# o1-labs/proof-systems

Hardware: AMD Instinct MI355X
Metric: MSM Mscalar/s at 2^20 (Vesta) (higher is better)
Workload: dtype u29x9 / u32x8 (255-bit Montgomery integers); 1 GPU; msm_2^20_vesta_srs; points_per_gpu=1048576, points_total=1048576, bases=SRS::<Vesta>::create, scalars=uniform 254-bit, seed 1234+rank, parallelism=point-range x1, world_size_seen=1

## Files before the change

proof_systems_amd/csrc/common.hpp:

```cpp
#pragma once
#include <hip/hip_runtime.h>
#include <stdarg.h>
#include <stdint.h>
#include <stdio.h>
#include <atomic>
#include <chrono>
#include <condition_variable>
#include <initializer_list>
#include <map>
#include <mutex>
#include <set>
#include <string>
#include <thread>
#include <vector>

#include "../../include/kimchi_hip.h"

namespace kh {

void set_error(const char* fmt, ...);

#define KH_HIP(expr)                                                                         \
    do {                                                                                     \
        hipError_t e_ = (expr);                                                              \
// ... 38 lines not shown
    hipEvent_t k0 = nullptr, k1 = nullptr;
    const char* kname = nullptr;
    hipEvent_t ev[MAXP + 1];
    const char* names[MAXP];
    int n = 0;
    bool created = false;
    bool enabled = false;
    int init() {
        if (created) return KH_OK;
        for (int i = 0; i <= MAXP; i++) KH_HIP(hipEventCreate(&ev[i]));
        KH_HIP(hipEventCreate(&k0)); KH_HIP(hipEventCreate(&k1));
        created = true;
        return KH_OK;
    }
    void begin(hipStream_t s) { n = 0; kname = nullptr; if (enabled && created) (void)hipEventRecord(ev[0], s); }
    void mark(const char* name, hipStream_t s) {
        if (!enabled || !created || n >= MAXP) return;
        names[n] = name; n++;
        (void)hipEventRecord(ev[n], s);
    }
};

struct MsmBasis {
    const void* pts = nullptr;
    const uint8_t* inf = nullptr;
    size_t n = 0;
    int precomp_c = 0;
    size_t stride = 0;
    size_t batch_stride = 0;
    const void* wide_pts = nullptr;
    int wide_c = 0;
    bool glv = false;
};

struct MsmJob {
    MsmBasis basis;
    size_t offset = 0;
    const uint64_t* scalars = nullptr;
    size_t n = 0, k = 0;
    int mont = 0, curve = 0;
    int W = 0, c = 0, precomp = 0, planes = 0, plane_shift[2] = {0, 0};
    int wide_lo = 0;
    size_t ngroups = 0;
    bool done_by_flag = false;
    bool fused = false, spread = false;
    bool spread_rerun = false;
};

struct MsmSlot {
    hipStream_t stream = nullptr;
    PhaseTimer timer;
    DevBuf ws_scalars, ws_digits, ws_hist, ws_cnt, ws_off, ws_ntask, ws_toff, ws_entries, ws_partial,
        ws_buckets, ws_seg, ws_out, ws_scan_tmp, ws_biglist, ws_points, ws_order, ws_chunks, ws_handed, ws_sync, ws_mid,
        ws_b29, ws_a1, ws_a2, ws_xlist;
    void* pinned = nullptr; size_t pinned_cap = 0;
    hipEvent_t done = nullptr;
    bool busy = false;
    std::thread::id owner;
    uint64_t ticket = 0;
    MsmJob job;
    volatile uint32_t* host_abort = nullptr;
    volatile uint32_t* spread_abort = nullptr;
    bool flag_unavailable = false;
    bool pinned_coherent = false;
    volatile uint32_t* done_flag = nullptr;
    DevBuf ws_done;
    uint32_t done_expect = 0;
};
static constexpr int MSM_SLOTS = 4;

struct Context {
    std::mutex mu;
    std::condition_variable cv;
    int sync_inflight = 0;
    std::multiset<std::thread::id> blocked_owners;
    int device = -1;
    bool ready = false;
    hipStream_t stream = nullptr;
    bool main_dirty = false;
    hipEvent_t order_ev = nullptr;
    int num_cus = 256;
    size_t lds_per_cu = (size_t)160 << 10, lds_per_block = (size_t)64 << 10;
    bool fused_disabled = false;
    PhaseTimer timer;
    std::vector<std::pair<const char*, float>> last;
    MsmSlot slot[MSM_SLOTS];
    uint64_t next_ticket = 1;
    std::chrono::steady_clock::time_point last_sync_msm_arrival{};
    DevBuf ws_ntt_a, ws_ntt_b;
    void* pinned = nullptr; size_t pinned_cap = 0;
    char* stage = nullptr; size_t stage_cap = 0, stage_cur = 0;
    int stage_upload(void* dst_dev, std::initializer_list<std::pair<const void*, size_t>> parts);
    void mark_async() { if (hipEventRecord(order_ev, stream) == hipSuccess) main_dirty = true; }
    std::mutex scratch_mu;
    std::map<std::string, DevBuf> scratch_bufs;
    std::set<std::string> done_flags;
    DevBuf& scratch(const char* name) { std::lock_guard<std::mutex> lk(scratch_mu); return scratch_bufs[name]; }
    bool once(const char* name) { std::lock_guard<std::mutex> lk(scratch_mu); return done_flags.insert(name).second; }
    void trim_scratch() { std::lock_guard<std::mutex> lk(scratch_mu); for (auto& kv : scratch_bufs) kv.second.release(); }
};
static constexpr int KH_MAX_DEVICES = 16;

Context& ctx();
int ensure_init();
struct DeviceScope {
    int prev;
    explicit DeviceScope(int device);
// ... 11 lines not shown
```

proof_systems_amd/csrc/context.hip:

```cpp
#include <stdlib.h>
#include <algorithm>
#include <atomic>

#include "api_internal.hpp"
#include "env.hpp"

namespace kh {

static thread_local std::string g_err;
void set_error(const char* fmt, ...) {
    char buf[1024];
    va_list ap; va_start(ap, fmt); vsnprintf(buf, sizeof(buf), fmt, ap); va_end(ap);
    g_err = buf;
}

static Context* g_ctx[KH_MAX_DEVICES];
static std::mutex g_ctx_mu;
static int g_default_dev = -1;
static thread_local int tl_dev = -1;
static thread_local int tl_hip_dev = -1;

static thread_local Context* tl_private[KH_MAX_DEVICES];
static std::vector<Context*> g_private_pool[KH_MAX_DEVICES];
static std::atomic<int> g_private_made[KH_MAX_DEVICES];
// ... 174 lines not shown
    return tl.e[d];
}

namespace {
struct DevPool {
    std::mutex mu;
    struct Block { void* p; kh::Context* owner; };
    std::multimap<size_t, Block> free_blocks[KH_MAX_DEVICES];
    std::map<void*, std::pair<int, size_t>> live;
    size_t cached[KH_MAX_DEVICES] = {0};
};
DevPool& dev_pool() { static DevPool p; return p; }
size_t pool_limit() { static const size_t lim = (size_t)env_int("KH_POOL_MAX_MB", 2048) << 20; return lim; }
}
static void dev_pool_trim(int device) {
    DevPool& P = dev_pool();
    std::lock_guard<std::mutex> lk(P.mu);
    const int d = device >= 0 && device < KH_MAX_DEVICES ? device : 0;
    for (auto& kv : P.free_blocks[d]) (void)hipFree(kv.second.p);
    P.free_blocks[d].clear(); P.cached[d] = 0;
}

extern "C" {

int kh_device_count(void) {
    int count = 0;
    if (hipGetDeviceCount(&count) != hipSuccess) return 0;
    return count;
}
int kh_init(int device_id) {
    int rc = do_init(device_id); if (rc) return rc;
    if (device_id >= 0) tl_dev = device_id;
    return KH_OK;
}
int kh_set_device(int device_id) {
    KH_REQUIRE(device_id >= 0, "kh_set_device: negative device id");
    int rc = do_init(device_id); if (rc) return rc;
    tl_dev = device_id;
    return KH_OK;
}
int kh_get_device(void) { return current_device(); }
int kh_trim(void) {
    int rc = ensure_init(); if (rc) return rc;
    Context& C = ctx();
    std::lock_guard<std::mutex> lk(C.mu);
    for (int i = 0; i < MSM_SLOTS; i++) {
        KH_REQUIRE(!C.slot[i].busy, "kh_trim: an MSM is in flight (kh_msm_wait first)");
        KH_HIP(hipStreamSynchronize(C.slot[i].stream));
    }
    for (int i = 0; i < MSM_SLOTS; i++) {
        MsmSlot& S = C.slot[i];
        for (DevBuf* b : {&S.ws_scalars, &S.ws_digits, &S.ws_hist, &S.ws_cnt, &S.ws_off, &S.ws_ntask, &S.ws_toff, &S.ws_entries, &S.ws_partial, &S.ws_buckets,
                          &S.ws_seg, &S.ws_out, &S.ws_scan_tmp, &S.ws_biglist, &S.ws_points, &S.ws_order, &S.ws_chunks, &S.ws_handed, &S.ws_sync, &S.ws_mid,
                          &S.ws_b29, &S.ws_a1, &S.ws_a2, &S.ws_xlist}) b->release();
    }
    C.ws_ntt_a.release(); C.ws_ntt_b.release();
    xfer_trim(C.device);
    dev_pool_trim(C.device);
    C.trim_scratch();
    {
        std::lock_guard<std::mutex> lk2(g_ctx_mu);
        if (g_private_active[C.device >= 0 && C.device < KH_MAX_DEVICES ? C.device : 0] == 0) ntt_trim(C);
    }
    return KH_OK;
}

int kh_private_context_begin(void) {
    int rc = ensure_init(); if (rc) return rc;
    const int dev = current_device();
    KH_REQUIRE(dev >= 0 && dev < KH_MAX_DEVICES, "no current device");
    KH_REQUIRE(!tl_private[dev], "kh_private_context_begin: this thread already has a private context on device %d", dev);
    Context& S = shared_ctx_of(dev);
    Context* c = tl_ctx_cache.c[dev];
    tl_ctx_cache.c[dev] = nullptr;
    if (!c) {
        std::lock_guard<std::mutex> lk(g_ctx_mu);
        if (!g_private_pool[dev].empty()) { c = g_private_pool[dev].back(); g_private_pool[dev].pop_back(); }
    }
    if (!c) {
        c = new (std::nothrow) Context;
        KH_REQUIRE(c, "out of memory");
        g_private_made[dev]++;
    }
    auto give_back = [&](int status) { std::lock_guard<std::mutex> lk(g_ctx_mu); g_private_pool[dev].push_back(c); return status; };
    if ((rc = bind_thread(dev)) || (rc = init_context(*c, dev))) return give_back(rc);
    {
        std::lock_guard<std::mutex> lk(S.mu);
        hipError_t e = hipEventRecord(S.order_ev, S.stream);
        if (e == hipSuccess) e = hipStreamWaitEvent(c->stream, S.order_ev, 0);
        if (e != hipSuccess) { set_error("kh_private_context_begin: ordering behind the shared context failed: %s", hipGetErrorString(e)); return give_back(KH_E_DEVICE); }
    }
    c->mark_async();
    tl_private[dev] = c;
    { std::lock_guard<std::mutex> lk(g_ctx_mu); g_private_active[dev]++; }
    return KH_OK;
}
int kh_set_phase_timers(int on) {
    int rc = ensure_init(); if (rc) return rc;
    Context& C = ctx();
    std::lock_guard<std::mutex> lk(C.mu);
    C.timer.enabled = on != 0; C.timer.n = 0;
    for (int i = 0; i < MSM_SLOTS; i++) { C.slot[i].timer.enabled = on != 0; C.slot[i].timer.n = 0; }
    return KH_OK;
}
int kh_private_context_active(void) {
    const int dev = current_device();
    return dev >= 0 && dev < KH_MAX_DEVICES && tl_private[dev] != nullptr;
// ... 183 lines not shown
```

proof_systems_amd/csrc/msm.hip:

```cpp
#include <hip/hip_ext.h>
#include <math.h>
#include "common.hpp"
#include "env.hpp"
#include "curve.cuh"
#include "coop.cuh"
#include "field29.cuh"
#include "host_ec.hpp"
#include "msm.hpp"
#include <condition_variable>
#include <functional>
#include <memory>
#include <thread>

namespace kh {

#define KH_HIGH_PRIO() __builtin_amdgcn_s_setprio(3)

class HostHelper {
    std::thread th_; std::mutex m_; std::condition_variable cv_, done_cv_;
    std::function<void()> job_; bool has_job_ = false, busy_ = false, stop_ = false;
    void loop() {
        std::unique_lock<std::mutex> lk(m_);
        for (;;) {
            cv_.wait(lk, [&] { return has_job_ || stop_; });
// ... 1257 lines not shown
    }
}
template <class BF>
__global__ void __launch_bounds__(128)
k_marginal_fin_q(const uint8_t* __restrict__ marg, MargGeom g, uint8_t* __restrict__ out, u32* __restrict__ done_ws, u32* __restrict__ done_flag) {
    KH_HIGH_PRIO();
    __shared__ u32 sh[32 * 32];
    const u32 j = blockIdx.x; const size_t q = blockIdx.y;
    const u32 v = threadIdx.x >> 2, role = threadIdx.x & 3u, f = g.wd[j];
    Fe<BF> r = Fe<BF>::zero();
    if (v < (1u << f)) r = quad_load<BF>(marg + ((q * 3 + j) * 32 + v) * 128);
    auto put = [&](const Fe<BF>& x) {
#pragma unroll
        for (int k = 0; k < 8; k++) sh[(v * 4 + role) * 8 + k] = x.v[k];
    };
    auto get = [&](u32 from) {
        Fe<BF> o = Fe<BF>::zero();
        if (from < 32) {
#pragma unroll
            for (int k = 0; k < 8; k++) o.v[k] = sh[(from * 4 + role) * 8 + k];
        }
        return o;
    };
    for (u32 d = 1; d < 32; d <<= 1) {
        put(r); __syncthreads();
        const Fe<BF> o = get(v + d);
        __syncthreads();
        r = quad_add<BF>(r, o);
    }
    if (v == 0 && j != 0) r = Fe<BF>::zero();
    for (u32 d = 16; d >= 1; d >>= 1) {
        put(r); __syncthreads();
        const Fe<BF> o = v < d ? get(v + d) : Fe<BF>::zero();
        __syncthreads();
        r = quad_add<BF>(r, o);
    }
    if (threadIdx.x < 4) quad_store<BF>(out + (q * 3 + j) * 128, r);
    if (done_ws) {
        __threadfence_system();
        __syncthreads();
        if (threadIdx.x == 0) {
            const u32 blocks = gridDim.x * gridDim.y;
            if (__hip_atomic_fetch_add(done_ws, 1u, __ATOMIC_ACQ_REL, __HIP_MEMORY_SCOPE_AGENT) == blocks - 1) {
                __hip_atomic_store(done_ws, 0u, __ATOMIC_RELAXED, __HIP_MEMORY_SCOPE_AGENT);
                const u32 e = done_ws[1] + 1;
                done_ws[1] = e;
                __threadfence_system();
                __hip_atomic_store(done_flag, e, __ATOMIC_RELEASE, __HIP_MEMORY_SCOPE_SYSTEM);
            }
        }
    }
}

struct WideGeom { u32 nb, lo, hi, rlog; };
template <class BF>
__global__ void __launch_bounds__(256)
k_bucket_sum_wide(const u32* __restrict__ toff, const u32* __restrict__ xlist, const u32* __restrict__ slist, const uint8_t* __restrict__ partial,
                  uint8_t* __restrict__ buckets29, u32 low, u32 SMALL_NT, u32* __restrict__ big, u32 cap, uint8_t* __restrict__ chunk_out) {
    KH_HIGH_PRIO();
    __shared__ __attribute__((aligned(16))) uint8_t total[4 * 128];
    const u32 count = xlist[1], nhot = big[0];
    for (u32 it = blockIdx.x * blockDim.x + threadIdx.x; it < count; it += gridDim.x * blockDim.x) {
        const u32 key = slist[it];
        const u32 t0 = toff[key], nt = toff[key + 1] - t0;
        if (nt > SMALL_NT) continue;
        Xyzz<BF> acc = Xyzz<BF>::load(partial + (size_t)t0 * 128);
        for (u32 k = 1; k < nt; k++) acc = add<BF>(acc, Xyzz<BF>::load(partial + (size_t)(t0 + k) * 128));
        uint8_t* const rec = buckets29 + (size_t)wide_true_bucket(key, low) * B29_BYTES;
        if (acc.is_identity()) store_b29_identity<BF>(rec); else store_b29<BF>(rec, xyzz_to29<BF>(acc));
    }
    if (nhot == 0) return;
    const u32 wave = threadIdx.x >> 6, lane = threadIdx.x & 63u, quad = lane >> 2;
    const u32 gw = blockIdx.x * (blockDim.x >> 6) + wave, GW = gridDim.x * (blockDim.x >> 6);
    u32 cbase = 0;
    for (u32 h = 0; h < nhot; h++) {
        const u32 key = big[2 + h];
        const u32 t0 = toff[key], nt = toff[key + 1] - t0, nch = (nt + CHUNK - 1) / CHUNK;
        for (u32 c = (gw + GW - cbase % GW) % GW; c < nch; c += GW) {
            const u32 lo = c * CHUNK, hi = lo + CHUNK < nt ? lo + CHUNK : nt;
            Fe<BF> acc = quad_identity<BF>();
            for (u32 k = lo + quad; k < hi; k += 16) acc = quad_add<BF>(acc, quad_load<BF>(partial + (size_t)(t0 + k) * 128));
            for (int d = 8; d >= 1; d >>= 1) acc = quad_add<BF>(acc, quad_shfl_down<BF>(acc, d));
            if (lane < 4) quad_store<BF>(chunk_out + (size_t)(cbase + c) * 128, acc);
            __threadfence();
            u32 arrived = 0;
            if (lane == 0) arrived = __hip_atomic_fetch_add(&big[2 + cap + h], 1u, __ATOMIC_ACQ_REL, __HIP_MEMORY_SCOPE_AGENT) + 1u;
            arrived = __shfl(arrived, 0, 64);
            if (arrived == nch) {
                __threadfence();
                Fe<BF> o = quad_identity<BF>();
                for (u32 k = quad; k < nch; k += 16) o = quad_add<BF>(o, quad_load<BF>(chunk_out + (size_t)(cbase + k) * 128));
                for (int d = 8; d >= 1; d >>= 1) o = quad_add<BF>(o, quad_shfl_down<BF>(o, d));
                if (lane < 4) quad_store<BF>(total + 128 * wave, o);
                __builtin_amdgcn_wave_barrier();
                if (lane == 0) {
                    const Xyzz<BF> v = Xyzz<BF>::load(total + 128 * wave);
                    uint8_t* const rec = buckets29 + (size_t)wide_true_bucket(key, low) * B29_BYTES;
                    if (v.is_identity()) store_b29_identity<BF>(rec); else store_b29<BF>(rec, xyzz_to29<BF>(v));
                }
                __builtin_amdgcn_wave_barrier();
            }
        }
        cbase += nch;
    }
}
__device__ __forceinline__ void wide_a1_item(const WideGeom& g, u32 out, u32& t0, u32& tstride) {
    const u32 per = g.nb >> g.rlog;
    if (out < per) { t0 = out << g.rlog; tstride = 1u; return; }
    const u32 cpm = (1u << g.hi) >> g.rlog, v = out - per, b = v / cpm, s = v - b * cpm;
    t0 = ((s << g.rlog) << g.lo) + b; tstride = 1u << g.lo;
}
template <class F>
__device__ __forceinline__ bool is_marker29(const Acc29<F>& a) { return a.zz.v[0] == 0xffffffffu; }
template <class BF>
__global__ void __launch_bounds__(256)
k_wide_a1(const uint8_t* __restrict__ buckets29, WideGeom g, u32 ngroups, uint8_t* __restrict__ out29) {
    KH_HIGH_PRIO();
    const u32 per = g.nb >> g.rlog, items = 2u * per;
    const u32 gid = blockIdx.x * blockDim.x + threadIdx.x;
    if (gid >= items * ngroups) return;
    const u32 q = gid / items, u = gid - q * items;
    u32 out = u;
    if (u >= per) { const u32 v = u - per, b = v & ((1u << g.lo) - 1u), sc = v >> g.lo; out = per + b * ((1u << g.hi) >> g.rlog) + sc; }
    u32 t0, ts;
    wide_a1_item(g, out, t0, ts);
    const uint8_t* B = buckets29 + ((size_t)q * g.nb + t0) * B29_BYTES;
    Acc29<BF> acc;
    bool have = false, ok = true;
    const u32 r = 1u << g.rlog;
#pragma unroll 1
    for (u32 i = 0; i < r; i++) {
        const Acc29<BF> b = load_b29<BF>(B + (size_t)i * ts * B29_BYTES);
        if (is_identity29<BF>(b)) continue;
        if (!have) { acc = b; have = true; continue; }
        ok = add29<BF>(acc, b);
        if (!ok) break;
    }
    uint8_t* o = out29 + ((size_t)q * items + out) * B29_BYTES;
    if (!ok) { acc.zz.v[0] = 0xffffffffu; store_b29<BF>(o, acc); return; }
    if (have) store_b29<BF>(o, acc); else store_b29_identity<BF>(o);
}
template <class BF>
__device__ __attribute__((noinline)) Xyzz<BF> wide_chunk_exact(const uint8_t* __restrict__ buckets29g, WideGeom g, u32 out) {
    u32 t0, ts;
    wide_a1_item(g, out, t0, ts);
    Xyzz<BF> acc = Xyzz<BF>::identity();
    const u32 r = 1u << g.rlog;
    for (u32 i = 0; i < r; i++) {
        const Acc29<BF> b = load_b29<BF>(buckets29g + ((size_t)t0 + (size_t)i * ts) * B29_BYTES);
        if (!is_identity29<BF>(b)) acc = add<BF>(acc, xyzz_from29<BF>(b));
    }
    return acc;
}
template <class BF>
__global__ void __launch_bounds__(64)
k_wide_a2(const uint8_t* __restrict__ in29, const uint8_t* __restrict__ buckets29, WideGeom g, uint8_t* __restrict__ outw) {
    KH_HIGH_PRIO();
    __shared__ u32 stage[32][64];
    const u32 slot = blockIdx.x, q = blockIdx.y, plane = slot >> g.lo, sidx = slot & ((1u << g.lo) - 1u);
    const u32 per = g.nb >> g.rlog, items = 2u * per;
    const u32 lane = threadIdx.x, role = lane & 3u, quad = lane >> 2;
    uint8_t* o = outw + (((size_t)q * 2 + plane) * (1u << g.lo) + sidx) * 128;
    u32 cnt, first;
    if (plane == 0) {
        const u32 a = sidx + 1u;
        if (a >= (1u << g.hi)) { if (lane < 4) quad_store<BF>(o, Fe<BF>::zero()); return; }
        cnt = (1u << g.lo) >> g.rlog; first = a * cnt;
    } else { cnt = (1u << g.hi) >> g.rlog; first = per + sidx * cnt; }
    const uint8_t* src = in29 + ((size_t)q * items + first) * B29_BYTES;
    Xyzz<BF> a = Xyzz<BF>::identity();
    for (u32 k = lane; k < cnt; k += 64) {
        const Acc29<BF> b = load_b29<BF>(src + (size_t)k * B29_BYTES);
        if (__builtin_expect(is_marker29<BF>(b), 0)) a = add<BF>(a, wide_chunk_exact<BF>(buckets29 + (size_t)q * g.nb * B29_BYTES, g, first + k));
        else if (!is_identity29<BF>(b)) a = add<BF>(a, xyzz_from29<BF>(b));
    }
#pragma unroll
    for (int k = 0; k < 8; k++) { stage[k][lane] = a.x.v[k]; stage[8 + k][lane] = a.y.v[k]; stage[16 + k][lane] = a.zz.v[k]; stage[24 + k][lane] = a.zzz.v[k]; }
    __syncthreads();
    auto parked = [&](u32 point) {
        Fe<BF> r;
#pragma unroll
        for (int k = 0; k < 8; k++) r.v[k] = stage[role * 8 + k][point];
        return r;
    };
    Fe<BF> acc = parked(quad);
    for (u32 k = 1; k < 4; k++) acc = quad_add<BF>(acc, parked(quad + 16 * k));
    for (int d = 8; d >= 1; d >>= 1) acc = quad_add<BF>(acc, quad_shfl_down<BF>(acc, d));
    if (lane < 4) quad_store<BF>(o, acc);
}

template <class BF>
__global__ void __launch_bounds__(256)
k_precompute(uint8_t* __restrict__ tables, const uint8_t* __restrict__ inf, size_t n, int c, int W, uint8_t* __restrict__ scratch) {
    size_t i = (size_t)blockIdx.x * blockDim.x + threadIdx.x;
    if (i >= n) return;
    if (inf && inf[i]) {
        for (int w = 1; w < W; w++) { Fe<BF> z = Fe<BF>::zero(); z.store(tables + ((size_t)w * n + i) * 64); z.store(tables + ((size_t)w * n + i) * 64 + 32); }
        return;
    }
    Xyzz<BF> P = Xyzz<BF>::from_affine(Aff<BF>::load(tables + i * 64));
    Fe<BF> prod = Fe<BF>::one();
    for (int w = 1; w < W; w++) {
        for (int k = 0; k < c; k++) P = dbl<BF>(P);
        P.store(scratch + ((size_t)(w - 1) * n + i) * 128);
        prod = mul<BF>(prod, P.zzz);
        prod.store(tables + ((size_t)w * n + i) * 64);
    }
    Fe<BF> iv = inv<BF>(prod);
    for (int w = W - 1; w >= 1; w--) {
        Xyzz<BF> Q = Xyzz<BF>::load(scratch + ((size_t)(w - 1) * n + i) * 128);
        Fe<BF> izzz = iv;
        if (w > 1) izzz = mul<BF>(iv, Fe<BF>::load(tables + ((size_t)(w - 1) * n + i) * 64));
        iv = mul<BF>(iv, Q.zzz);
        Fe<BF> izz = sqr<BF>(mul<BF>(izzz, Q.zz));
        Fe<BF> x = mul<BF>(Q.x, izz), y = mul<BF>(Q.y, izzz);
        x.store(tables + ((size_t)w * n + i) * 64);
        y.store(tables + ((size_t)w * n + i) * 64 + 32);
    }
}

struct VestaCfg { typedef FqParams Base; typedef FpParams Scalar; };
struct PallasCfg { typedef FpParams Base; typedef FqParams Scalar; };

static std::atomic<size_t>& wide_min_n_cell() {
    static std::atomic<size_t> v{(size_t)env_int("KH_WIDE_MIN_N", 1 << 19)};
    return v;
}
static std::atomic<u32>& sort_staging_cell(int i) {
    static std::atomic<u32> v[2] = {{(u32)env_int("KH_PART2_STAGE", 28672)}, {(u32)env_int("KH_PART2_MAXPASS", 2)}};
    return v[i];
}
void msm_set_sort_staging(unsigned entries, unsigned max_passes) { sort_staging_cell(0).store(entries); sort_staging_cell(1).store(max_passes); }
size_t msm_wide_min_n() { const size_t v = wide_min_n_cell().load(); return v ? v : ~(size_t)0; }
void msm_set_wide_min_n(size_t n) { wide_min_n_cell().store(n); }
int msm_pick_window(size_t n) {
    int lg = 0; while (((size_t)1 << (lg + 1)) <= n) lg++;
    int c = lg - 3;
    if (c < 4) c = 4;
    if (c > 16) c = 16;
    return c;
}
// ... 26 lines not shown
}

template <class CFG>
static int msm_enqueue_t(Context& Ctx, MsmSlot& C, const MsmBasis& basis, size_t offset, const u64* scalars_dev, size_t n, size_t k,
                         int mont, int curve, int flags) {
    typedef typename CFG::Base BF; typedef typename CFG::Scalar SF;
    hipStream_t s = C.stream;
    const bool wide = basis.wide_pts && basis.wide_c > 16 && basis.wide_c - 9 <= (int)PART2_MAXLOW && n >= msm_wide_min_n() && k <= 4 &&
                      (size_t)windows_of(basis.wide_c) * n <= ((size_t)1 << 26);
    static constexpr u32 SPREAD_MAX_NT = 256;
    const void* const tab_pts = wide ? basis.wide_pts : basis.pts;
    const int c = wide ? basis.wide_c : (basis.precomp_c ? basis.precomp_c : msm_pick_window(n));
    const bool glv = basis.glv && !wide && basis.precomp_c != 0;
    const int W = glv ? 2 * ((128 + c - 1) / c) : windows_of(c);
    const u32 nb = 1u << (c - 1);
    const int precomp = (wide || basis.precomp_c) ? 1 : 0;
    int S = (int)(n / 32768); if (S < 1) S = 1; if (S > 16) S = 16;
    { int want = (int)(512 / ((size_t)W * k)); if (want < 1) want = 1; if (S > want) S = want; }
    const size_t tab_stride = basis.stride ? basis.stride : basis.n;
    SortGeom g{n, nb, S, W, precomp, tab_stride, offset, basis.batch_stride};
    const size_t ngroups = precomp ? k : k * (size_t)W;
    const bool few_groups = ngroups <= 8;
    const bool quad_sum = !wide && precomp && few_groups;
    const bool spread = quad_sum && (flags & MSM_SPREAD_SCALARS) != 0;
    const int Sq = precomp ? W * S : S;
    const size_t nkeys = ngroups * nb;
    const size_t M = n * (size_t)W * k;
    const size_t cap = (size_t)Ctx.num_cus * 256 * 4;
    size_t room_sz = cap / 4;
    if (nkeys < cap / 2) room_sz = cap - cap / 16 - nkeys / 2;
    const u32 room = (u32)room_sz;
    const u32 kmin = 8;
    const KTab ktab = precomp ? task_length_table(nkeys, (u32)Ctx.num_cus) : KTab{};
    const size_t max_tasks = M / 4 + nkeys + 1;
    KH_REQUIRE(M < ((size_t)1 << 31) && (tab_stride * (size_t)(precomp ? W : 1) + basis.batch_stride * k) < ((size_t)1 << 31), "MSM too large for 31-bit entry indices (n=%zu k=%zu)", n, k);

    int rc;
    if ((rc = C.ws_digits.reserve(M * sizeof(int32_t)))) return rc;
    if ((rc = C.ws_hist.reserve(nkeys * Sq * sizeof(u32)))) return rc;
    if ((rc = C.ws_cnt.reserve((nkeys + 2) * sizeof(u32)))) return rc;
    if ((rc = C.ws_off.reserve((nkeys + 2) * sizeof(u32)))) return rc;
    if ((rc = C.ws_ntask.reserve((nkeys + 2) * sizeof(u32)))) return rc;
    if ((rc = C.ws_toff.reserve((nkeys + 2) * sizeof(u32)))) return rc;
    if ((rc = C.ws_entries.reserve((M + 1) * sizeof(u32)))) return rc;
    if ((rc = C.ws_partial.reserve(max_tasks * 128))) return rc;
    if ((rc = C.ws_handed.reserve((max_tasks + 2) * sizeof(u32)))) return rc;
    if ((rc = C.ws_buckets.reserve(nkeys * 128))) return rc;
    const size_t bigcap = nkeys + max_tasks / CHUNK + 2;
    if ((rc = C.ws_biglist.reserve((2 + 4 * bigcap) * sizeof(u32)))) return rc;
    if ((rc = C.ws_chunks.reserve(bigcap * 128))) return rc;
    if ((rc = C.ws_order.reserve((2 * (MAX_K + 1) + 3 * (nkeys + 2)) * sizeof(u32)))) return rc;
    WideGeom wg{};
    static constexpr u32 wide_og = 16, wide_acc_blocks = 3, wide_rlog = 4;
    static_assert((wide_og & (wide_og - 1)) == 0 && wide_og <= (1u << (17 - 9)) && wide_rlog >= 1 && wide_rlog <= 17 / 2, "wide-path constants");
    size_t wide_acc_lds = (Ctx.lds_per_cu / (wide_acc_blocks + 1) + 1024) & ~(size_t)1023;
    if (wide_acc_lds > Ctx.lds_per_block) wide_acc_lds = Ctx.lds_per_block & ~(size_t)1023;
    if (wide) {
        if ((rc = C.ws_xlist.reserve((3 * max_tasks + 8) * sizeof(u32)))) return rc;
        if ((rc = C.ws_handed.reserve((2 * max_tasks + 4) * sizeof(u32)))) return rc;
        wg.nb = nb; wg.lo = (u32)c / 2; wg.hi = (u32)(c - 1) - wg.lo; wg.rlog = wide_rlog;
        if ((rc = C.ws_b29.reserve(nkeys * B29_BYTES))) return rc;
        if ((rc = C.ws_a1.reserve(ngroups * 2 * (size_t)(nb >> wg.rlog) * B29_BYTES))) return rc;
        if ((rc = C.ws_a2.reserve(ngroups * 2 * ((size_t)1 << wg.lo) * 128))) return rc;
    }
    u32 m = 1;
    while (m < 16 && (ngroups * (size_t)nb) / m > 65536) m <<= 1;
    if (!precomp && m < 4) m = 4;
    if (nb < m) m = nb;
    const u32 nseg = nb / m;
    const u32 nblk1 = (nseg + SUM_BLK - 1) / SUM_BLK;
    const u32 planes = wide ? 3u : ((precomp && ngroups <= 4096 && c >= 7 && c <= 16) ? 3u : 0u);
    MargGeom mg{};
    if (planes) {
        const u32 bits = wide ? wg.lo : (u32)c - 1, f0 = (bits + 2) / 3, f1 = (bits - f0 + 1) / 2, f2 = bits - f0 - f1;
        mg.nb = wide ? 1u << wg.lo : nb; mg.sh[0] = 0; mg.wd[0] = f0; mg.sh[1] = f0; mg.wd[1] = f1; mg.sh[2] = f0 + f1; mg.wd[2] = f2;
    }
    const size_t tail_groups = wide ? 2 * ngroups : ngroups;
    const size_t nout = planes ? tail_groups * planes : ngroups;
    if ((rc = C.ws_seg.reserve(std::max(ngroups * (size_t)(nseg + nblk1), nout * (size_t)32) * 128))) return rc;
    if ((rc = C.ws_out.reserve(nout * 128))) return rc;
    if (C.pinned_cap < nout * 128) {
        if (C.pinned) (void)hipHostFree(C.pinned);
        C.pinned = nullptr; C.pinned_cap = 0;
        C.pinned_coherent = hipHostMalloc(&C.pinned, nout * 128 + 4096, hipHostMallocCoherent | hipHostMallocMapped) == hipSuccess;
        if (!C.pinned_coherent) { (void)hipGetLastError(); C.pinned = nullptr; KH_HIP(hipHostMalloc(&C.pinned, nout * 128 + 4096, hipHostMallocDefault)); }
        C.pinned_cap = nout * 128 + 4096;
    }
    if (Ctx.once("msm_attr")) {
        KH_HIP(hipFuncSetAttribute((const void*)k_hist, hipFuncAttributeMaxDynamicSharedMemorySize, 131072));
        KH_HIP(hipFuncSetAttribute((const void*)k_scatter, hipFuncAttributeMaxDynamicSharedMemorySize, 131072));
        KH_HIP(hipFuncSetAttribute((const void*)k_sort_fused, hipFuncAttributeMaxDynamicSharedMemorySize, 131072));
    }
    static const bool fused_off = env_flag("KH_NO_FUSED_SORT", false);
    static const unsigned long long fused_spin_ticks = 100ull * (unsigned long long)env_int("KH_FUSED_SPIN_US", 20000);
    FusedGeom fg{};
    bool fused = precomp && !wide && !fused_off && !Ctx.fused_disabled && k <= 4 && M < ((size_t)1 << 22) && nb >= 2048 && Ctx.num_cus >= 128;
    if (fused) {
        fg.n = (u32)n; fg.nb = nb; fg.W = (u32)W; fg.k = (u32)k; fg.bpg = (u32)std::min<size_t>(FUSED_G, FUSED_B / (2 * k)); fg.nkeys = (u32)nkeys;
        fg.split = 2; fg.sub = nb / fg.split;
        fg.room = room; fg.kmin = kmin; fg.ktab = ktab; fg.pt_stride = tab_stride; fg.pt_offset = offset; fg.pt_batch = basis.batch_stride;
        const size_t threads = (size_t)fg.bpg * k * fg.split * FUSED_T;
        fg.kpt = (u32)((nkeys + 1 + threads - 1) / threads);
        const size_t tot4 = (size_t)W * n / 4, chunk4 = (tot4 + fg.bpg - 1) / fg.bpg + 1;
        if (fg.kpt > (u32)FUSED_KPT || n < 4 || ((size_t)W * n) % 4 || chunk4 > (size_t)FUSED_V * FUSED_T || fg.sub > (u32)FUSED_C * FUSED_T) fused = false;
    }
    const bool part = wide || (precomp && !fused && nb == ((u32)PART_P << PART_LOW) && n <= ((size_t)1 << 20) && W <= 16 && M >= ((size_t)1 << 21));
    const u32 part_low = wide ? (u32)c - 9 : (u32)PART_LOW;
    const u32 part_nblk = wide ? (u32)std::max<size_t>(std::max<size_t>(1, std::min<size_t>(256, 512 / k)), ((size_t)W * n + 65535) / 65536)
                               : (part ? (u32)std::max<size_t>(1, std::min<size_t>(256, 512 / k)) : 0);
    const size_t part_size = (size_t)k * PART_P * part_nblk;
    if (part) {
        if ((rc = C.ws_hist.reserve((part_size + 1) * sizeof(u32)))) return rc;
        if ((rc = C.ws_cnt.reserve((part_size + 1) * sizeof(u32)))) return rc;
        if ((rc = C.ws_mid.reserve(M * sizeof(u32)))) return rc;
    }
// ... 106 lines not shown
    const u32 acc_prio = (flags & MSM_LATENCY) ? 1u : 0u;
    uint8_t* const b29 = wide ? C.ws_b29.as<uint8_t>() : nullptr;
    if (wide) {
        const dim3 wgrid((unsigned)(nkeys / 256));
        auto kern = k_acc_wide29<BF>;
        if (C.timer.enabled && C.timer.created) {
            hipExtLaunchKernelGGL(kern, wgrid, dim3(256), wide_acc_lds, s, C.timer.k0, C.timer.k1, 0, C.ws_entries.as<u32>(), C.ws_off.as<u32>(), C.ws_toff.as<u32>(), order, (u32)nkeys,
                                  (const uint8_t*)tab_pts, C.ws_partial.as<uint8_t>(), b29, part_low, C.ws_handed.as<u32>());
            C.timer.kname = "k_acc_wide29";
        } else
        hipLaunchKernelGGL(kern, wgrid, dim3(256), wide_acc_lds, s, C.ws_entries.as<u32>(), C.ws_off.as<u32>(), C.ws_toff.as<u32>(), order, (u32)nkeys,
                           (const uint8_t*)tab_pts, C.ws_partial.as<uint8_t>(), b29, part_low, C.ws_handed.as<u32>());
        const unsigned xgrid = M / nkeys >= 64 ? 2048u : WIDE_XB;
        hipLaunchKernelGGL((k_acc_wide_rest<BF>), dim3(xgrid), dim3(256), 0, s, C.ws_entries.as<u32>(), C.ws_off.as<u32>(), C.ws_toff.as<u32>(), C.ws_xlist.as<u32>(),
                           C.ws_handed.as<u32>(), (const uint8_t*)tab_pts, C.ws_partial.as<uint8_t>(), b29, part_low);
    } else {
        auto kern = k_accumulate29<BF>;
        if (C.timer.enabled && C.timer.created) {
            hipExtLaunchKernelGGL(kern, agrid, dim3(256), 0, s, C.timer.k0, C.timer.k1, 0,
                                  C.ws_entries.as<u32>(), C.ws_off.as<u32>(), C.ws_toff.as<u32>(), roff, order, nkeys,
                                  (const uint8_t*)tab_pts, C.ws_partial.as<uint8_t>(), C.ws_handed.as<u32>(), abort_dev, acc_prio);
            C.timer.kname = "k_accumulate29";
        } else
        hipLaunchKernelGGL(kern, agrid, dim3(256), 0, s,
                           C.ws_entries.as<u32>(), C.ws_off.as<u32>(), C.ws_toff.as<u32>(), roff, order, nkeys,
                           (const uint8_t*)tab_pts, C.ws_partial.as<uint8_t>(), C.ws_handed.as<u32>(), abort_dev, acc_prio);
    }
    C.timer.mark("accumulate", s);
    if (wide)
        hipLaunchKernelGGL((k_bucket_sum_wide<BF>), dim3(256), dim3(256), 0, s, C.ws_toff.as<u32>(), C.ws_xlist.as<u32>(), C.ws_xlist.as<u32>() + 2 + 2 * max_tasks,
                           C.ws_partial.as<uint8_t>(), b29, part_low, WIDE_HOT_NT, C.ws_biglist.as<u32>(), (u32)bigcap, C.ws_chunks.as<uint8_t>());
    else if (quad_sum)
        hipLaunchKernelGGL((k_bucket_sum_q<BF>), dim3((unsigned)((4 * nkeys + 255) / 256)), dim3(256), 0, s,
                           C.ws_toff.as<u32>(), nkeys, C.ws_partial.as<uint8_t>(), C.ws_buckets.as<uint8_t>(), C.ws_biglist.as<u32>(),
                           bigcap, spread ? SPREAD_MAX_NT : 16u, abort_dev, spread ? (u32*)C.spread_abort : nullptr);
    else
    hipLaunchKernelGGL((k_bucket_sum<BF>), dim3((unsigned)((nkeys + 255) / 256)), dim3(256), 0, s,
                       C.ws_toff.as<u32>(), nkeys, C.ws_partial.as<uint8_t>(), C.ws_buckets.as<uint8_t>(), C.ws_biglist.as<u32>(),
                       bigcap, nkeys <= 16384 ? 4u : 16u, abort_dev);
    if (!wide && !spread) {
    hipLaunchKernelGGL((k_bucket_chunk<BF>), dim3(2048), dim3(64), 0, s,
                       C.ws_toff.as<u32>(), C.ws_partial.as<uint8_t>(), C.ws_biglist.as<u32>(), bigcap, C.ws_chunks.as<uint8_t>(), abort_dev);
    hipLaunchKernelGGL((k_bucket_big<BF>), dim3(1024), dim3(256), 0, s,
                       C.ws_toff.as<u32>(), C.ws_chunks.as<uint8_t>(), C.ws_buckets.as<uint8_t>(), C.ws_biglist.as<u32>(), bigcap, abort_dev);
    }
    C.timer.mark("bucket_sum", s);
    u32* const done_ws = flag_on ? C.ws_done.as<u32>() : nullptr; u32* const done_flag = flag_on ? (u32*)C.done_flag : nullptr;
    if (flag_on) C.done_expect++;
    bool direct_out = false;
    if (wide) {
        const u32 items = 2u * (nb >> wg.rlog) * (u32)ngroups;
        hipLaunchKernelGGL((k_wide_a1<BF>), dim3((items + 255) / 256), dim3(256), 0, s, b29, wg, (u32)ngroups, C.ws_a1.as<uint8_t>());
        C.timer.mark("reduce_a1", s);
        hipLaunchKernelGGL((k_wide_a2<BF>), dim3(2u << wg.lo, (unsigned)ngroups), dim3(64), 0, s, C.ws_a1.as<uint8_t>(), b29, wg, C.ws_a2.as<uint8_t>());
        hipLaunchKernelGGL((k_marginals_q<BF>), dim3(32, 3, (unsigned)tail_groups), dim3(256), 0, s, C.ws_a2.as<uint8_t>(), mg, C.ws_seg.as<uint8_t>());
        hipLaunchKernelGGL((k_marginal_fin_q<BF>), dim3(3, (unsigned)tail_groups), dim3(128), 0, s, C.ws_seg.as<uint8_t>(), mg, (uint8_t*)C.pinned, done_ws, done_flag);
        direct_out = true;
    } else if (planes) {
        if ((mg.nb >> mg.wd[0]) >= 256)
            hipLaunchKernelGGL((k_marginals_h<BF>), dim3(32, 3, (unsigned)ngroups), dim3(256), 0, s, C.ws_buckets.as<uint8_t>(), mg, C.ws_seg.as<uint8_t>());
        else if (few_groups)
            hipLaunchKernelGGL((k_marginals_q<BF>), dim3(32, 3, (unsigned)ngroups), dim3(256), 0, s, C.ws_buckets.as<uint8_t>(), mg, C.ws_seg.as<uint8_t>());
        else
            hipLaunchKernelGGL((k_marginals<BF>), dim3(32, 3, (unsigned)ngroups), dim3(64), 0, s, C.ws_buckets.as<uint8_t>(), mg, C.ws_seg.as<uint8_t>());
        static const bool fin_quad = !env_flag("KH_NO_FIN_QUAD", false);
        if (few_groups || fin_quad) {
            hipLaunchKernelGGL((k_marginal_fin_q<BF>), dim3(3, (unsigned)ngroups), dim3(128), 0, s, C.ws_seg.as<uint8_t>(), mg, (uint8_t*)C.pinned, done_ws, done_flag);
            direct_out = true;
        } else
            hipLaunchKernelGGL((k_marginal_fin<BF>), dim3(3, (unsigned)ngroups), dim3(64), 0, s, C.ws_seg.as<uint8_t>(), mg, C.ws_out.as<uint8_t>());
    } else {
    hipLaunchKernelGGL((k_reduce_seg<BF>), dim3((unsigned)((ngroups * nseg + 127) / 128)), dim3(128), 0, s,
                       C.ws_buckets.as<uint8_t>(), nb, m, ngroups, C.ws_seg.as<uint8_t>());
    {
        uint8_t* lvl1 = C.ws_seg.as<uint8_t>() + ngroups * (size_t)nseg * 128;
        hipLaunchKernelGGL((k_sum_level<BF>), dim3(nblk1, (unsigned)ngroups), dim3(256), 0, s, C.ws_seg.as<uint8_t>(), nseg, nblk1, lvl1);
        hipLaunchKernelGGL((k_sum_final<BF>), dim3((unsigned)ngroups), dim3(nblk1 > 64 ? 256 : 64), 0, s, lvl1, nblk1, C.ws_out.as<uint8_t>());
    }
    }
    C.timer.mark("reduce", s);
    KH_HIP(hipGetLastError());
    if (!direct_out) KH_HIP(hipMemcpyAsync(C.pinned, C.ws_out.p, nout * 128, hipMemcpyDeviceToHost, s));
    KH_HIP(hipEventRecord(C.done, s));
    C.busy = true; C.owner = std::this_thread::get_id(); C.ticket = Ctx.next_ticket++;
    C.job = {basis, offset, scalars_dev, n, k, mont, curve, W, c, precomp, (int)planes, {(int)mg.wd[0], (int)mg.wd[1]}, wide ? (int)wg.lo : 0, ngroups,
             direct_out && flag_on, fused, spread};
    return KH_OK;
}

int msm_enqueue(Context& C, MsmSlot& S, int curve, const MsmBasis& basis, size_t offset, const uint64_t* scalars_dev, size_t n, size_t k, int mont,
                int flags) {
    if (n == 0 || k == 0) {
        S.busy = true; S.owner = std::this_thread::get_id(); S.ticket = C.next_ticket++;
        S.job = {basis, offset, scalars_dev, n, k, mont, curve};
        KH_HIP(hipEventRecord(S.done, S.stream));
        return KH_OK;
    }
    if (curve == KH_CURVE_VESTA) return msm_enqueue_t<VestaCfg>(C, S, basis, offset, scalars_dev, n, k, mont, curve, flags);
    return msm_enqueue_t<PallasCfg>(C, S, basis, offset, scalars_dev, n, k, mont, curve, flags);
}

static int msm_rerun(Context& C, MsmSlot& S) {
    const MsmJob j = S.job;
    const uint64_t ticket = S.ticket; const auto owner = S.owner;
    int rc = msm_enqueue(C, S, j.curve, j.basis, j.offset, j.scalars, j.n, j.k, j.mont);
    S.ticket = ticket; S.owner = owner; C.next_ticket--;
    if (rc) { S.busy = false; return rc; }
// ... 196 lines not shown
```

Before: 1029 Mscalar/s.

## Add second-level 29-bit affine reduction stage before wide bucket a2 reduction

Inserts a new k_wide_l2 kernel that sums groups of 2^flog first-level partial sums in the cheap 29-bit affine form, so k_wide_a2 only has to combine a few run results per slot with XYZZ quad adds. k_wide_a2 is restructured so each block handles 16 runs and does a shuffle tree over them, falling back to exact recomputation through the chunks and buckets when a marker is hit. The aim is to move most of the reduction work from the expensive projective adds into batched affine adds with better parallelism. The cost is an extra kernel launch, an extra workspace buffer, and a more complex fallback path.

```diff
diff --git a/proof_systems_amd/csrc/common.hpp b/proof_systems_amd/csrc/common.hpp
--- a/proof_systems_amd/csrc/common.hpp
+++ b/proof_systems_amd/csrc/common.hpp
@@ -114,7 +114,7 @@
     PhaseTimer timer;
     DevBuf ws_scalars, ws_digits, ws_hist, ws_cnt, ws_off, ws_ntask, ws_toff, ws_entries, ws_partial,
         ws_buckets, ws_seg, ws_out, ws_scan_tmp, ws_biglist, ws_points, ws_order, ws_chunks, ws_handed, ws_sync, ws_mid,
-        ws_b29, ws_a1, ws_a2, ws_xlist;
+        ws_b29, ws_a1, ws_l2, ws_a2, ws_xlist;
     void* pinned = nullptr; size_t pinned_cap = 0;
     hipEvent_t done = nullptr;
     bool busy = false;
diff --git a/proof_systems_amd/csrc/context.hip b/proof_systems_amd/csrc/context.hip
--- a/proof_systems_amd/csrc/context.hip
+++ b/proof_systems_amd/csrc/context.hip
@@ -250,7 +250,7 @@
         MsmSlot& S = C.slot[i];
         for (DevBuf* b : {&S.ws_scalars, &S.ws_digits, &S.ws_hist, &S.ws_cnt, &S.ws_off, &S.ws_ntask, &S.ws_toff, &S.ws_entries, &S.ws_partial, &S.ws_buckets,
                           &S.ws_seg, &S.ws_out, &S.ws_scan_tmp, &S.ws_biglist, &S.ws_points, &S.ws_order, &S.ws_chunks, &S.ws_handed, &S.ws_sync, &S.ws_mid,
-                          &S.ws_b29, &S.ws_a1, &S.ws_a2, &S.ws_xlist}) b->release();
+                          &S.ws_b29, &S.ws_a1, &S.ws_l2, &S.ws_a2, &S.ws_xlist}) b->release();
     }
     C.ws_ntt_a.release(); C.ws_ntt_b.release();
     xfer_trim(C.device);
diff --git a/proof_systems_amd/csrc/msm.hip b/proof_systems_amd/csrc/msm.hip
--- a/proof_systems_amd/csrc/msm.hip
+++ b/proof_systems_amd/csrc/msm.hip
@@ -1333,7 +1333,7 @@
     }
 }
 
-struct WideGeom { u32 nb, lo, hi, rlog; };
+struct WideGeom { u32 nb, lo, hi, rlog, flog; };
 template <class BF>
 __global__ void __launch_bounds__(256)
 k_bucket_sum_wide(const u32* __restrict__ toff, const u32* __restrict__ xlist, const u32* __restrict__ slist, const uint8_t* __restrict__ partial,
@@ -1394,6 +1394,21 @@
 template <class F>
 __device__ __forceinline__ bool is_marker29(const Acc29<F>& a) { return a.zz.v[0] == 0xffffffffu; }
 template <class BF>
+__device__ __forceinline__ void wide_sum29(const uint8_t* __restrict__ in, size_t stride, u32 n, uint8_t* __restrict__ o) {
+    Acc29<BF> acc;
+    bool have = false, ok = true;
+#pragma unroll 1
+    for (u32 i = 0; i < n; i++) {
+        const Acc29<BF> b = load_b29<BF>(in + (size_t)i * stride);
+        if (is_identity29<BF>(b)) continue;
+        if (!have) { acc = b; have = true; ok = !is_marker29<BF>(b); }
+        else ok = !is_marker29<BF>(b) && add29<BF>(acc, b);
+        if (!ok) break;
+    }
+    if (!ok) { acc.zz.v[0] = 0xffffffffu; store_b29<BF>(o, acc); return; }
+    if (have) store_b29<BF>(o, acc); else store_b29_identity<BF>(o);
+}
+template <class BF>
 __global__ void __launch_bounds__(256)
 k_wide_a1(const uint8_t* __restrict__ buckets29, WideGeom g, u32 ngroups, uint8_t* __restrict__ out29) {
     KH_HIGH_PRIO();
@@ -1405,21 +1420,15 @@
     if (u >= per) { const u32 v = u - per, b = v & ((1u << g.lo) - 1u), sc = v >> g.lo; out = per + b * ((1u << g.hi) >> g.rlog) + sc; }
     u32 t0, ts;
     wide_a1_item(g, out, t0, ts);
-    const uint8_t* B = buckets29 + ((size_t)q * g.nb + t0) * B29_BYTES;
-    Acc29<BF> acc;
-    bool have = false, ok = true;
-    const u32 r = 1u << g.rlog;
-#pragma unroll 1
-    for (u32 i = 0; i < r; i++) {
-        const Acc29<BF> b = load_b29<BF>(B + (size_t)i * ts * B29_BYTES);
-        if (is_identity29<BF>(b)) continue;
-        if (!have) { acc = b; have = true; continue; }
-        ok = add29<BF>(acc, b);
-        if (!ok) break;
-    }
-    uint8_t* o = out29 + ((size_t)q * items + out) * B29_BYTES;
-    if (!ok) { acc.zz.v[0] = 0xffffffffu; store_b29<BF>(o, acc); return; }
-    if (have) store_b29<BF>(o, acc); else store_b29_identity<BF>(o);
+    wide_sum29<BF>(buckets29 + ((size_t)q * g.nb + t0) * B29_BYTES, (size_t)ts * B29_BYTES, 1u << g.rlog, out29 + ((size_t)q * items + out) * B29_BYTES);
+}
+template <class BF>
+__global__ void __launch_bounds__(256)
+k_wide_l2(const uint8_t* __restrict__ in29, u32 flog, u32 nrec, uint8_t* __restrict__ out29) {
+    KH_HIGH_PRIO();
+    const u32 gid = blockIdx.x * blockDim.x + threadIdx.x;
+    if (gid >= nrec) return;
+    wide_sum29<BF>(in29 + ((size_t)gid << flog) * B29_BYTES, B29_BYTES, 1u << flog, out29 + (size_t)gid * B29_BYTES);
 }
 template <class BF>
 __device__ __attribute__((noinline)) Xyzz<BF> wide_chunk_exact(const uint8_t* __restrict__ buckets29g, WideGeom g, u32 out) {
@@ -1434,40 +1443,46 @@
     return acc;
 }
 template <class BF>
+__device__ __attribute__((noinline)) Xyzz<BF> wide_run_exact(const uint8_t* __restrict__ chunks29g, const uint8_t* __restrict__ buckets29g, WideGeom g, u32 run) {
+    Xyzz<BF> acc = Xyzz<BF>::identity();
+    const u32 f = 1u << g.flog, c0 = run << g.flog;
+    for (u32 i = 0; i < f; i++) {
+        const Acc29<BF> b = load_b29<BF>(chunks29g + (size_t)(c0 + i) * B29_BYTES);
+        if (is_marker29<BF>(b)) acc = add<BF>(acc, wide_chunk_exact<BF>(buckets29g, g, c0 + i));
+        else if (!is_identity29<BF>(b)) acc = add<BF>(acc, xyzz_from29<BF>(b));
+    }
+    return acc;
+}
+template <class BF>
 __global__ void __launch_bounds__(64)
-k_wide_a2(const uint8_t* __restrict__ in29, const uint8_t* __restrict__ buckets29, WideGeom g, uint8_t* __restrict__ outw) {
-    KH_HIGH_PRIO();
-    __shared__ u32 stage[32][64];
-    const u32 slot = blockIdx.x, q = blockIdx.y, plane = slot >> g.lo, sidx = slot & ((1u << g.lo) - 1u);
-    const u32 per = g.nb >> g.rlog, items = 2u * per;
-    const u32 lane = threadIdx.x, role = lane & 3u, quad = lane >> 2;
-    uint8_t* o = outw + (((size_t)q * 2 + plane) * (1u << g.lo) + sidx) * 128;
-    u32 cnt, first;
-    if (plane == 0) {
-        const u32 a = sidx + 1u;
-        if (a >= (1u << g.hi)) { if (lane < 4) quad_store<BF>(o, Fe<BF>::zero()); return; }
-        cnt = (1u << g.lo) >> g.rlog; first = a * cnt;
-    } else { cnt = (1u << g.hi) >> g.rlog; first = per + sidx * cnt; }
-    const uint8_t* src = in29 + ((size_t)q * items + first) * B29_BYTES;
-    Xyzz<BF> a = Xyzz<BF>::identity();
-    for (u32 k = lane; k < cnt; k += 64) {
-        const Acc29<BF> b = load_b29<BF>(src + (size_t)k * B29_BYTES);
-        if (__builtin_expect(is_marker29<BF>(b), 0)) a = add<BF>(a, wide_chunk_exact<BF>(buckets29 + (size_t)q * g.nb * B29_BYTES, g, first + k));
-        else if (!is_identity29<BF>(b)) a = add<BF>(a, xyzz_from29<BF>(b));
-    }
-#pragma unroll
-    for (int k = 0; k < 8; k++) { stage[k][lane] = a.x.v[k]; stage[8 + k][lane] = a.y.v[k]; stage[16 + k][lane] = a.zz.v[k]; stage[24 + k][lane] = a.zzz.v[k]; }
-    __syncthreads();
-    auto parked = [&](u32 point) {
-        Fe<BF> r;
-#pragma unroll
-        for (int k = 0; k < 8; k++) r.v[k] = stage[role * 8 + k][point];
-        return r;
-    };
-    Fe<BF> acc = parked(quad);
-    for (u32 k = 1; k < 4; k++) acc = quad_add<BF>(acc, parked(quad + 16 * k));
-    for (int d = 8; d >= 1; d >>= 1) acc = quad_add<BF>(acc, quad_shfl_down<BF>(acc, d));
-    if (lane < 4) quad_store<BF>(o, acc);
+k_wide_a2(const uint8_t* __restrict__ runs29, const uint8_t* __restrict__ chunks29, const uint8_t* __restrict__ buckets29, WideGeom g, uint8_t* __restrict__ outw) {
+    KH_HIGH_PRIO();
+    __shared__ u32 stage[32][16];
+    const u32 q = blockIdx.y, lane = threadIdx.x, role = lane & 3u, quad = lane >> 2;
+    const u32 per = g.nb >> g.rlog, per2 = per >> g.flog;
+    const u32 r0 = blockIdx.x * 16u, plane = r0 >= per2 ? 1u : 0u;
+    const u32 s = ((1u << (plane ? g.hi : g.lo)) >> g.rlog) >> g.flog;
+    uint8_t* const og = outw + ((size_t)q * 2 + plane) * (1u << g.lo) * 128;
+    if (lane < 16) {
+        const u32 run = r0 + lane;
+        const Acc29<BF> b = load_b29<BF>(runs29 + ((size_t)q * 2 * per2 + run) * B29_BYTES);
+        Xyzz<BF> a = Xyzz<BF>::identity();
+        if (__builtin_expect(is_marker29<BF>(b), 0)) a = wide_run_exact<BF>(chunks29 + (size_t)q * 2 * per * B29_BYTES, buckets29 + (size_t)q * g.nb * B29_BYTES, g, run);
+        else if (!is_identity29<BF>(b)) a = xyzz_from29<BF>(b);
+#pragma unroll
+        for (int k = 0; k < 8; k++) { stage[k][lane] = a.x.v[k]; stage[8 + k][lane] = a.y.v[k]; stage[16 + k][lane] = a.zz.v[k]; stage[24 + k][lane] = a.zzz.v[k]; }
+    }
+    __syncthreads();
+    Fe<BF> acc;
+#pragma unroll
+    for (int k = 0; k < 8; k++) acc.v[k] = stage[role * 8 + k][quad];
+    for (u32 d = s >> 1; d >= 1; d >>= 1) acc = quad_add<BF>(acc, quad_shfl_down<BF>(acc, (int)d));
+    if ((quad & (s - 1u)) == 0u) {
+        const u32 m = (r0 - plane * per2 + quad) / s;
+        if (plane || m) quad_store<BF>(og + (size_t)(m - (plane ? 0u : 1u)) * 128, acc);
+    }
+    if (plane == 0 && lane < 4)
+        for (u32 p = (1u << g.hi) - 1u + blockIdx.x; p < (1u << g.lo); p += per2 / 16u) quad_store<BF>(og + (size_t)p * 128, Fe<BF>::zero());
 }
 
 template <class BF>
@@ -1600,15 +1615,17 @@
     if ((rc = C.ws_order.reserve((2 * (MAX_K + 1) + 3 * (nkeys + 2)) * sizeof(u32)))) return rc;
     WideGeom wg{};
     static constexpr u32 wide_og = 16, wide_acc_blocks = 3, wide_rlog = 4;
-    static_assert((wide_og & (wide_og - 1)) == 0 && wide_og <= (1u << (17 - 9)) && wide_rlog >= 1 && wide_rlog <= 17 / 2, "wide-path constants");
+    static_assert((wide_og & (wide_og - 1)) == 0 && wide_og <= (1u << (17 - 9)) && wide_rlog >= 1 && wide_rlog + 2 <= 17 / 2, "wide-path constants");
     size_t wide_acc_lds = (Ctx.lds_per_cu / (wide_acc_blocks + 1) + 1024) & ~(size_t)1023;
     if (wide_acc_lds > Ctx.lds_per_block) wide_acc_lds = Ctx.lds_per_block & ~(size_t)1023;
     if (wide) {
         if ((rc = C.ws_xlist.reserve((3 * max_tasks + 8) * sizeof(u32)))) return rc;
         if ((rc = C.ws_handed.reserve((2 * max_tasks + 4) * sizeof(u32)))) return rc;
         wg.nb = nb; wg.lo = (u32)c / 2; wg.hi = (u32)(c - 1) - wg.lo; wg.rlog = wide_rlog;
+        wg.flog = wg.lo > wg.rlog + 5 ? wg.lo - wg.rlog - 4 : 1;
         if ((rc = C.ws_b29.reserve(nkeys * B29_BYTES))) return rc;
         if ((rc = C.ws_a1.reserve(ngroups * 2 * (size_t)(nb >> wg.rlog) * B29_BYTES))) return rc;
+        if ((rc = C.ws_l2.reserve(ngroups * 2 * (size_t)(nb >> (wg.rlog + wg.flog)) * B29_BYTES))) return rc;
         if ((rc = C.ws_a2.reserve(ngroups * 2 * ((size_t)1 << wg.lo) * 128))) return rc;
     }
     u32 m = 1;
@@ -1821,7 +1838,10 @@
         const u32 items = 2u * (nb >> wg.rlog) * (u32)ngroups;
         hipLaunchKernelGGL((k_wide_a1<BF>), dim3((items + 255) / 256), dim3(256), 0, s, b29, wg, (u32)ngroups, C.ws_a1.as<uint8_t>());
         C.timer.mark("reduce_a1", s);
-        hipLaunchKernelGGL((k_wide_a2<BF>), dim3(2u << wg.lo, (unsigned)ngroups), dim3(64), 0, s, C.ws_a1.as<uint8_t>(), b29, wg, C.ws_a2.as<uint8_t>());
+        const u32 runs = 2u * (nb >> (wg.rlog + wg.flog)) * (u32)ngroups;
+        hipLaunchKernelGGL((k_wide_l2<BF>), dim3((runs + 63) / 64), dim3(64), 0, s, C.ws_a1.as<uint8_t>(), wg.flog, runs, C.ws_l2.as<uint8_t>());
+        hipLaunchKernelGGL((k_wide_a2<BF>), dim3(runs / (u32)ngroups / 16u, (unsigned)ngroups), dim3(64), 0, s, C.ws_l2.as<uint8_t>(), C.ws_a1.as<uint8_t>(), b29, wg,
+                           C.ws_a2.as<uint8_t>());
         hipLaunchKernelGGL((k_marginals_q<BF>), dim3(32, 3, (unsigned)tail_groups), dim3(256), 0, s, C.ws_a2.as<uint8_t>(), mg, C.ws_seg.as<uint8_t>());
         hipLaunchKernelGGL((k_marginal_fin_q<BF>), dim3(3, (unsigned)tail_groups), dim3(128), 0, s, C.ws_seg.as<uint8_t>(), mg, (uint8_t*)C.pinned, done_ws, done_flag);
         direct_out = true;
```

After: 1042 Mscalar/s (median of 6 runs). 1.01x the previous value.
